# Lukeasargen/Show-Attend-and-Tell-Pytorch-Lightning

Hardware: AMD Instinct MI355X
Metric: captions/sec (train step) at B=128, 256px, seq_len=22 (higher is better)
Workload: dtype bf16; 1 GPU; C2: resnet50 encoder_size=7 encoder_dim=512 vocab=6400 T=22, 128 images/GPU x R=5 captions, trainable encoder, Adam, full lengths, decoder_tf=always; global_batch_images=128, parallelism=dp1, grad_bucket_dtype=fp32

## Files before the change

show-attend-and-tell-pytorch-lightning_amd/csrc/api.hip:

```cpp
#include <stdarg.h>

#include "../../include/sat_hip.h"
#include "decoder.h"
#include "gemm.h"
#include "gemm_bf16_common.h"
#include "temperature.h"
#include "caption_score.h"

namespace sat {
static thread_local char g_err[512] = {0};
int& dev_switch(int which) {
    static int v[SW_COUNT] = {0 , getenv("SAT_NO_WGRAD3X3") ? !atoi(getenv("SAT_NO_WGRAD3X3")) : 1,
                              getenv("SAT_REDUCE_Z16") ? atoi(getenv("SAT_REDUCE_Z16")) : 1, getenv("SAT_WIDE_TILES") ? atoi(getenv("SAT_WIDE_TILES")) : 0,
                              getenv("SAT_BN_ONEPASS") ? atoi(getenv("SAT_BN_ONEPASS")) : 1,
                              getenv("SAT_BN_VPT") ? atoi(getenv("SAT_BN_VPT")) : 2,
                              getenv("SAT_ACC_PREFETCH") ? atoi(getenv("SAT_ACC_PREFETCH")) : 0};
    return v[which];
}
int& trace_launches() { static int on = getenv("SAT_TRACE_LAUNCH") ? 1 : 0; return on; }
char* last_error_buf() { return g_err; }
int fail(int code, const char* fmt, ...) {
    va_list ap; va_start(ap, fmt); vsnprintf(g_err, sizeof g_err, fmt, ap); va_end(ap);
    return code;
}
}

using namespace sat;

extern "C" {

int sat_abi_version(void) { return SAT_HIP_ABI_VERSION; }
int sat_debug_trace_launches(int32_t on) { sat::trace_launches() = on ? 1 : 0; return SAT_OK; }
int sat_debug_option(const char* name, int32_t value) {
    if (!name) return fail(SAT_EINVAL, "debug_option: null name");
    if (!strcmp(name, "wgrad3x3")) { dev_switch(SW_WGRAD3X3) = value; return SAT_OK; }
    if (!strcmp(name, "reduce_z16")) { dev_switch(SW_REDUCE_Z16) = value; return SAT_OK; }
    if (!strcmp(name, "acc_prefetch")) { dev_switch(SW_ACC_PREFETCH) = value; return SAT_OK; }
    if (!strcmp(name, "bn_vpt")) { dev_switch(SW_BN_VPT) = value; return SAT_OK; }
    if (!strcmp(name, "bn_onepass")) { dev_switch(SW_BN_ONEPASS) = value; return SAT_OK; }
    if (!strcmp(name, "wide_tiles")) { dev_switch(SW_WIDE_TILES) = value; return SAT_OK; }
    if (!strcmp(name, "glds_tile")) { glds_force_tile() = value; return SAT_OK; }
    if (!strcmp(name, "glds_stages8")) { glds_stages8() = value; return SAT_OK; }
    if (!strcmp(name, "glds_tall_k")) { glds_tall_k() = value; return SAT_OK; }
    if (!strcmp(name, "glds_tall_conv")) { glds_tall_conv() = value; return SAT_OK; }
    if (!strcmp(name, "tile_override")) { gemm_tile_override() = value; return SAT_OK; }
    return fail(SAT_EINVAL, "debug_option: unknown option %s", name);
}
const char* sat_last_error(void) { return last_error_buf(); }

static int gemm_from_desc(const sat_gemm_desc* d, const sat_gemm_types* t, void* stream);
int sat_gemm_f32(const sat_gemm_desc* d, void* stream) { return gemm_from_desc(d, nullptr, stream); }
int sat_gemm_ex(const sat_gemm_desc* d, const sat_gemm_types* t, void* stream) {
    if (!t) return fail(SAT_EINVAL, "sat_gemm_ex: null type descriptor");
    return gemm_from_desc(d, t, stream);
}
static int gemm_from_desc(const sat_gemm_desc* d, const sat_gemm_types* t, void* stream) {
    if (!d) return fail(SAT_EINVAL, "sat_gemm_f32: null descriptor");
    if (d->amode != A_ROW && d->amode != A_KMAJOR) return fail(SAT_EINVAL, "sat_gemm_f32: amode %d (dense modes only)", d->amode);
    if (d->bmode != B_ROW && d->bmode != B_KMAJOR) return fail(SAT_EINVAL, "sat_gemm_f32: bmode %d (dense modes only)", d->bmode);
    GemmArgs g;
    g.A = d->A; g.lda = d->lda; g.a_rows = d->a_rows; g.B = d->B; g.ldb = d->ldb; g.C = d->C; g.ldc = d->ldc; g.c_rows = d->c_rows;
    g.M = d->M; g.N = d->N; g.K = d->K; g.amode = d->amode; g.bmode = d->bmode; g.accumulate = d->accumulate; g.epi = d->epi;
    g.bias = d->bias; g.e0 = d->e0; g.lde0 = d->lde0; g.c0 = d->c0; g.c1 = d->c1; g.slab = d->slab; g.slab_elems = d->slab_elems;
    if (t) { g.a_bf16 = t->a_bf16; g.b_bf16 = t->b_bf16; g.c_bf16 = t->c_bf16; g.bf16_mfma = t->bf16_mfma; }
    return launch_gemm(g, (hipStream_t)stream);
}

size_t sat_decoder_workspace_bytes(const sat_decoder_dims* d) {
    if (check_dims(d) != SAT_OK) return 0;
    return decoder_workspace_bytes(*d);
}

static int check_params(const sat_decoder_dims* d, const sat_decoder_params* w, const char* what) {
    if (!w) return fail(SAT_EINVAL, "%s: null parameter struct", what);
    if (!w->embedding || !w->init_f_w || !w->init_f_b || !w->init_i_w || !w->init_i_b || !w->w_ih || !w->w_hh || !w->b_ih || !w->b_hh ||
        !w->att_enc || !w->att_dec || !w->att_f || !w->beta_w || !w->beta_b || !w->out_hidden || !w->out_w)
        return fail(SAT_EINVAL, "%s: null tensor in parameter struct", what);
    if (d->deep_output && !w->out_context) return fail(SAT_EINVAL, "%s: deep output needs output.context.weight", what);
    for (int l = 1; l < d->layers; ++l)
        if (!w->up_w_ih[l - 1] || !w->up_w_hh[l - 1] || !w->up_b_ih[l - 1] || !w->up_b_hh[l - 1])
            return fail(SAT_EINVAL, "%s: null tensor for LSTM layer %d", what, l);
    return SAT_OK;
}
static int check_batch(const sat_decoder_batch* b) {
    if (!b || !b->ann || !b->caps || !b->lengths || !b->prow || !b->src_row || !b->step_offsets_host || !b->teacher_host)
        return fail(SAT_EINVAL, "decoder: null field in batch struct");
    return SAT_OK;
}

int sat_decoder_train_fwd(const sat_decoder_dims* d, const sat_decoder_params* w, const sat_decoder_batch* b, float* logits_packed,
                          float* alphas, void* workspace, size_t workspace_bytes, void* stream) {
    SAT_TRY(check_dims(d)); SAT_TRY(check_params(d, w, "decoder_train_fwd")); SAT_TRY(check_batch(b));
    if (!alphas || !workspace || (d->P > 0 && !logits_packed)) return fail(SAT_EINVAL, "decoder_train_fwd: null output/workspace");
    return decoder_fwd(*d, *w, *b, logits_packed, alphas, (char*)workspace, workspace_bytes, (hipStream_t)stream);
}

int sat_decoder_train_bwd(const sat_decoder_dims* d, const sat_decoder_params* w, const sat_decoder_batch* b, const float* dlogits_packed,
                          const float* alphas, const float* dalphas, const sat_decoder_params* g, float* dann, void* workspace,
                          size_t workspace_bytes, void* stream) {
    SAT_TRY(check_dims(d)); SAT_TRY(check_params(d, w, "decoder_train_bwd")); SAT_TRY(check_params(d, g, "decoder_train_bwd(grads)")); SAT_TRY(check_batch(b));
    if (!alphas || !dann || !workspace || (d->P > 0 && !dlogits_packed)) return fail(SAT_EINVAL, "decoder_train_bwd: null input/output/workspace");
    return decoder_bwd(*d, *w, *b, dlogits_packed, alphas, dalphas, *g, dann, (char*)workspace, workspace_bytes, (hipStream_t)stream);
}

int sat_ce_label_smooth_fwd(const float* logits, const int32_t* targets, int32_t P, int32_t V, float smoothing, float* lse_rows,
                            float* loss_rows, int32_t* correct_rows, float* out, void* stream) {
    if (!logits || !targets || !lse_rows || !loss_rows || !correct_rows || !out) return fail(SAT_EINVAL, "ce_label_smooth_fwd: null pointer");
    return ce_fwd(logits, targets, P, V, smoothing, lse_rows, loss_rows, correct_rows, out, (hipStream_t)stream);
}
int sat_ce_label_smooth_bwd(const float* logits, const int32_t* targets, const float* lse_rows, int32_t P, int32_t V, float smoothing,
                            const float* gscale, float* dlogits, void* stream) {
    if (!logits || !targets || !lse_rows || !dlogits) return fail(SAT_EINVAL, "ce_label_smooth_bwd: null pointer");
    return ce_bwd(logits, targets, lse_rows, P, V, smoothing, gscale, dlogits, (hipStream_t)stream);
}
int sat_doubly_stochastic_fwd(const float* alphas, int32_t N, int32_t T1, int32_t L, float gamma, float* asum, float* part, float* out, void* stream) {
    if (!alphas || !asum || !part || !out) return fail(SAT_EINVAL, "doubly_stochastic_fwd: null pointer");
    return ds_fwd(alphas, N, T1, L, gamma, asum, part, out, (hipStream_t)stream);
}
int sat_doubly_stochastic_bwd(const float* asum, const float* gscale, int32_t N, int32_t T1, int32_t L, float gamma, float* dalphas, void* stream) {
    if (!asum || !dalphas) return fail(SAT_EINVAL, "doubly_stochastic_bwd: null pointer");
    return ds_bwd(asum, gscale, N, T1, L, gamma, dalphas, (hipStream_t)stream);
}

size_t sat_temperature_workspace_bytes(int32_t P, int32_t V) {
    if (P <= 0 || V <= 0) { fail(SAT_EINVAL, "temperature_workspace_bytes: non-positive size (P=%d V=%d)", P, V); return 0; }
    return temperature_workspace_bytes(P, V);
}
int sat_temperature_nll(const float* logits, const int32_t* targets, int32_t P, int32_t V, const float* temperatures, int32_t n_temperatures,
// ... 460 lines not shown
```

show-attend-and-tell-pytorch-lightning_amd/csrc/encoder.hip:

```cpp
#include <stdlib.h>
#include "../../include/sat_hip.h"
#include "common.h"
#include "gemm.h"
#include "profile.h"

namespace sat {

typedef __bf16 bf16x4 __attribute__((ext_vector_type(4)));
template <typename T> __device__ __forceinline__ float4 ld4(const T* p, long i4);
template <> __device__ __forceinline__ float4 ld4<float>(const float* p, long i4) { return reinterpret_cast<const float4*>(p)[i4]; }
template <> __device__ __forceinline__ float4 ld4<__bf16>(const __bf16* p, long i4) {
    bf16x4 v = reinterpret_cast<const bf16x4*>(p)[i4];
    return make_float4((float)v[0], (float)v[1], (float)v[2], (float)v[3]);
}
template <typename T> __device__ __forceinline__ void st4(T* p, long i4, float4 v);
template <> __device__ __forceinline__ void st4<float>(float* p, long i4, float4 v) { reinterpret_cast<float4*>(p)[i4] = v; }
template <> __device__ __forceinline__ void st4<__bf16>(__bf16* p, long i4, float4 v) {
    bf16x4 o; o[0] = (__bf16)v.x; o[1] = (__bf16)v.y; o[2] = (__bf16)v.z; o[3] = (__bf16)v.w;
    reinterpret_cast<bf16x4*>(p)[i4] = o;
}

__global__ void cast_f32_bf16_kernel(const float* __restrict__ src, __bf16* __restrict__ dst, long n4) {
    long e = (long)blockIdx.x * blockDim.x + threadIdx.x;
    if (e < n4) st4<__bf16>(dst, e, reinterpret_cast<const float4*>(src)[e]);
}
__global__ void normalize_nhwc8_bf16_kernel(const float* __restrict__ img, __bf16* __restrict__ out, int H, int W, long total,
                                            float m0, float m1, float m2, float s0, float s1, float s2) {
    long e = (long)blockIdx.x * blockDim.x + threadIdx.x;
    if (e >= total) return;
    long hw = (long)H * W; long n = e / hw, p = e - n * hw;
    const float* src = img + n * 3 * hw + p;
    st4<__bf16>(out, 2 * e, make_float4((src[0] - m0) / s0, (src[hw] - m1) / s1, (src[2 * hw] - m2) / s2, 0.f));
    st4<__bf16>(out, 2 * e + 1, make_float4(0.f, 0.f, 0.f, 0.f));
}
__global__ void pad_c3_to_c8_bf16_kernel(const float* __restrict__ w3, __bf16* __restrict__ w8, long n) {
    long e = (long)blockIdx.x * blockDim.x + threadIdx.x;
    if (e >= n) return;
    st4<__bf16>(w8, 2 * e, make_float4(w3[3 * e], w3[3 * e + 1], w3[3 * e + 2], 0.f));
    st4<__bf16>(w8, 2 * e + 1, make_float4(0.f, 0.f, 0.f, 0.f));
}
__global__ void unpad_c8_to_c3_kernel(const float* __restrict__ w8, float* __restrict__ w3, long n) {
    long e = (long)blockIdx.x * blockDim.x + threadIdx.x;
    if (e >= n) return;
    w3[3 * e] = w8[8 * e]; w3[3 * e + 1] = w8[8 * e + 1]; w3[3 * e + 2] = w8[8 * e + 2];
}

__global__ void normalize_nhwc4_padded_bf16_kernel(const float* __restrict__ img, __bf16* __restrict__ out, int H, int W, long total,
                                                   float m0, float m1, float m2, float s0, float s1, float s2) {
    long e = (long)blockIdx.x * blockDim.x + threadIdx.x;
    if (e >= total) return;
    const int Wp = W + 6, Hp = H + 6;
    const unsigned eu = (unsigned)e;
    const int xp = (int)(eu % Wp); const unsigned t = eu / Wp; const int yp = (int)(t % Hp); const long n = t / Hp;
    const int x = xp - 3, y = yp - 3;
    float4 v = make_float4(0.f, 0.f, 0.f, 0.f);
    if ((unsigned)x < (unsigned)W && (unsigned)y < (unsigned)H) {
        const long hw = (long)H * W; const float* src = img + n * 3 * hw + (long)y * W + x;
        v = make_float4((src[0] - m0) / s0, (src[hw] - m1) / s1, (src[2 * hw] - m2) / s2, 0.f);
    }
    st4<__bf16>(out, e, v);
}
__global__ void stem_filter_pairs_kernel(const float* __restrict__ w3, __bf16* __restrict__ wp, long n) {
    long e = (long)blockIdx.x * blockDim.x + threadIdx.x;
    if (e >= n) return;
    const int sp = (int)(e % 4); const long kr = e / 4;
    const float* a = w3 + (kr * 7 + 2 * sp) * 3;
    st4<__bf16>(wp, 2 * e, make_float4(a[0], a[1], a[2], 0.f));
    st4<__bf16>(wp, 2 * e + 1, sp < 3 ? make_float4(a[3], a[4], a[5], 0.f) : make_float4(0.f, 0.f, 0.f, 0.f));
}
__global__ void stem_filter_grad_unpairs_kernel(const float* __restrict__ dwp, float* __restrict__ dw3, long n) {
    long e = (long)blockIdx.x * blockDim.x + threadIdx.x;
    if (e >= n) return;
    const int s = (int)(e % 7); const long kr = e / 7;
    const float* a = dwp + ((kr * 4 + (s >> 1)) * 8 + (s & 1) * 4);
    dw3[3 * e] = a[0]; dw3[3 * e + 1] = a[1]; dw3[3 * e + 2] = a[2];
}

__global__ void normalize_nhwc4_kernel(const float* __restrict__ img, float* __restrict__ out, int H, int W, long total,
                                       float m0, float m1, float m2, float s0, float s1, float s2) {
    long e = (long)blockIdx.x * blockDim.x + threadIdx.x;
    if (e >= total) return;
    long hw = (long)H * W; long n = e / hw, p = e - n * hw;
    const float* src = img + n * 3 * hw + p;
    float4 v;
    v.x = (src[0] - m0) / s0; v.y = (src[hw] - m1) / s1; v.z = (src[2 * hw] - m2) / s2; v.w = 0.f;
    reinterpret_cast<float4*>(out)[e] = v;
// ... 740 lines not shown
    if (V == 4) reinterpret_cast<float4*>(y)[e] = make_float4(s[0], s[1], s[2], s[3]);
    else y[e] = s[0];
}
__device__ __forceinline__ void bilinear_src(int o, int in, int out, int& i0, int& i1, float& l1) {
    float s = ((float)o + 0.5f) * ((float)in / (float)out) - 0.5f;
    if (s < 0.f) s = 0.f;
    i0 = (int)s; i1 = i0 + (i0 < in - 1 ? 1 : 0); l1 = s - (float)i0;
}
__global__ void bilinear_fwd_kernel(const float* __restrict__ x, float* __restrict__ y, int H, int W, int C, int P, int Q, long total) {
    long e = (long)blockIdx.x * blockDim.x + threadIdx.x;
    if (e >= total) return;
    const unsigned eu = (unsigned)e; int c = (int)(eu % C); unsigned t = eu / C; int q = (int)(t % Q); t /= Q; int p = (int)(t % P); long n = t / P;
    int h0, h1, w0, w1; float lh, lw;
    bilinear_src(p, H, P, h0, h1, lh); bilinear_src(q, W, Q, w0, w1, lw);
    const float* b = x + n * H * W * C + c;
    float v00 = b[((long)h0 * W + w0) * C], v01 = b[((long)h0 * W + w1) * C], v10 = b[((long)h1 * W + w0) * C], v11 = b[((long)h1 * W + w1) * C];
    y[e] = (1.f - lh) * ((1.f - lw) * v00 + lw * v01) + lh * ((1.f - lw) * v10 + lw * v11);
}
__global__ void bilinear_bwd_kernel(const float* __restrict__ dy, float* __restrict__ dx, int H, int W, int C, int P, int Q, long total) {
    long e = (long)blockIdx.x * blockDim.x + threadIdx.x;
    if (e >= total) return;
    const unsigned eu = (unsigned)e; int c = (int)(eu % C); unsigned t = eu / C; int w = (int)(t % W); t /= W; int h = (int)(t % H); long n = t / H;
    float s = 0.f;
    for (int p = 0; p < P; ++p) {
        int h0, h1; float lh; bilinear_src(p, H, P, h0, h1, lh);
        float wh = (h0 == h ? 1.f - lh : 0.f) + (h1 == h ? lh : 0.f);
        if (wh == 0.f) continue;
        for (int q = 0; q < Q; ++q) {
            int w0, w1; float lw; bilinear_src(q, W, Q, w0, w1, lw);
            float ww = (w0 == w ? 1.f - lw : 0.f) + (w1 == w ? lw : 0.f);
            if (ww != 0.f) s += wh * ww * dy[((n * P + p) * Q + q) * C + c];
        }
    }
    dx[e] = s;
}

template <typename T>
__global__ void grouped_filter_expand_kernel(const T* __restrict__ wg, T* __restrict__ wd, int K, int C, int RS, int groups) {
    const long e = (long)blockIdx.x * blockDim.x + threadIdx.x;
    const long total = (long)K * RS * C;
    if (e >= total) return;
    const int c = (int)(e % C); const long t = e / C; const int rs = (int)(t % RS), k = (int)(t / RS);
    const int cg = C / groups, kg = K / groups;
    const int g = k / kg;
    const int cl = c - g * cg;
    wd[e] = (cl >= 0 && cl < cg) ? wg[((long)k * RS + rs) * cg + cl] : (T)0.f;
}
__global__ void grouped_filter_grad_extract_kernel(const float* __restrict__ dwd, float* __restrict__ dwg, int K, int C, int RS, int groups) {
    const long e = (long)blockIdx.x * blockDim.x + threadIdx.x;
    const int cg = C / groups, kg = K / groups;
    const long total = (long)K * RS * cg;
    if (e >= total) return;
    const int cl = (int)(e % cg); const long t = e / cg; const int rs = (int)(t % RS), k = (int)(t / RS);
    dwg[e] = dwd[((long)k * RS + rs) * C + (k / kg) * cg + cl];
}

}

using namespace sat;

static int conv_geom(const sat_conv_geom* g, ConvGeom& o, int vec = 4) {
    SAT_REQUIRE(g, "conv: null geometry");
    o.N = g->N; o.H = g->H; o.W = g->W; o.C = g->C; o.K = g->K; o.R = g->R; o.S = g->S; o.stride = g->stride; o.pad = g->pad; o.sw = (g->stride_w > 0 && g->stride_w != g->stride) ? g->stride_w : 0;
    SAT_REQUIRE(o.N > 0 && o.H > 0 && o.W > 0 && o.C > 0 && o.K > 0 && o.R > 0 && o.S > 0 && o.stride > 0 && o.pad >= 0, "conv: bad geometry");
    o.P = (o.H + 2 * o.pad - o.R) / o.stride + 1; o.Q = (o.W + 2 * o.pad - o.S) / (o.sw ? o.sw : o.stride) + 1;
    SAT_REQUIRE(o.P > 0 && o.Q > 0, "conv: empty output");
    SAT_REQUIRE(o.C % vec == 0 && o.K % vec == 0, "conv: C=%d and K=%d must be multiples of %d (pad the stem channels)", o.C, o.K, vec);
    return SAT_OK;
}

extern "C" {

static int conv_fwd_any(const void* x, const void* w, const float* bias, void* y, const sat_conv_geom* geom, int bf16, void* stream,
                        float* tile_stats = nullptr, int* tile_rows = nullptr) {
    ConvGeom g; SAT_TRY(conv_geom(geom, g, bf16 ? 8 : 4));
    if (!x || !w || !y) return fail(SAT_EINVAL, "conv2d_fwd: null pointer");
    GemmArgs a; a.a_bf16 = a.b_bf16 = a.c_bf16 = a.bf16_mfma = bf16;
    a.M = g.N * g.P * g.Q; a.N = g.K; a.K = g.R * g.S * g.C;
    a.B = w; a.ldb = a.K; a.bmode = B_ROW; a.C = y; a.ldc = g.K; a.g = g;
    if (g.R == 1 && g.S == 1 && g.stride == 1 && g.pad == 0) { a.A = x; a.lda = g.C; a.amode = A_ROW; }
    else { a.A = x; a.amode = A_CONV_FWD; }
    if (bias) { a.epi = EPI_BIAS; a.bias = bias; }
    a.tile_stats = tile_stats; a.tile_rows = tile_rows;
    return launch_gemm(a, (hipStream_t)stream);
}
int sat_conv2d_fwd(const float* x, const float* w, const float* bias, float* y, const sat_conv_geom* geom, void* stream) {
    return conv_fwd_any(x, w, bias, y, geom, 0, stream);
}
int sat_conv2d_fwd_bf16(const void* x, const void* w, const float* bias, void* y, const sat_conv_geom* geom, void* stream) {
    return conv_fwd_any(x, w, bias, y, geom, 1, stream);
}
size_t sat_conv2d_fwd_stats_bytes(const sat_conv_geom* geom) {
    ConvGeom g; if (conv_geom(geom, g, 8) != SAT_OK) return 0;
    return (size_t)cdiv((long)g.N * g.P * g.Q, 64L) * g.K * 2 * sizeof(float);
}
int sat_conv2d_fwd_bf16_stats(const void* x, const void* w, void* y, const sat_conv_geom* geom, float* tile_stats, int32_t* tile_rows, void* stream) {
    if (!tile_stats || !tile_rows) return fail(SAT_EINVAL, "conv2d_fwd_bf16_stats: null statistics buffer");
    int tr = 0;
    SAT_TRY(conv_fwd_any(x, w, nullptr, y, geom, 1, stream, tile_stats, &tr));
    *tile_rows = tr;
    return SAT_OK;
}

struct BnBwdStats { const void* x; const unsigned char* mask; const float* mean; const float* invstd; float* tile_stats; int* tile_rows; };
static int conv_dgrad_any(const void* dy, const void* w, void* dx, const sat_conv_geom* geom, int accumulate, int bf16, void* stream,
                          const BnBwdStats* bs = nullptr, const void* add_src = nullptr, const uint8_t* add_mask = nullptr) {
    ConvGeom g; SAT_TRY(conv_geom(geom, g, bf16 ? 8 : 4));
    if (!dy || !w || !dx) return fail(SAT_EINVAL, "conv2d_dgrad: null pointer");
    GemmArgs a; a.a_bf16 = a.b_bf16 = a.c_bf16 = a.bf16_mfma = bf16;
    a.accumulate = accumulate; a.C = dx; a.ldc = g.C; a.g = g;
    if (add_src) {
        SAT_REQUIRE(bf16 && g.stride == 1, "conv2d_dgrad: add_src needs bf16 storage and stride 1");
        a.accumulate = 1; a.add_src = add_src; a.add_mask = add_mask;
    }
    if (bs) {
        *bs->tile_rows = 0;
        if (bf16 && !(g.stride == 2)) {
            a.bn_x = bs->x; a.bn_mask = bs->mask; a.bn_mean = bs->mean; a.bn_invstd = bs->invstd; a.tile_stats = bs->tile_stats; a.tile_rows = bs->tile_rows;
        }
    }
    if (g.R == 1 && g.S == 1 && g.stride == 1 && g.pad == 0) {
        a.M = g.N * g.H * g.W; a.N = g.C; a.K = g.K; a.A = dy; a.lda = g.K; a.amode = A_ROW; a.B = w; a.ldb = g.C; a.bmode = B_KMAJOR;
    } else if (bf16 && g.stride == 2) {
        a.A = dy; a.amode = A_CONV_DGRAD; a.B = w; a.bmode = B_CONV_DGRAD_W; a.N = g.C;
        for (int ph = 0; ph < 2; ++ph)
            for (int pw = 0; pw < 2; ++pw) {
                ConvGeom c = g; c.cls = 1; c.ph = ph; c.pw = pw;
                c.Hc = (g.H - ph + 1) / 2; c.Wc = (g.W - pw + 1) / 2;
                c.r0 = (ph + g.pad) & 1; c.s0 = (pw + g.pad) & 1;
                c.rc = c.r0 < g.R ? (g.R - c.r0 + 1) / 2 : 0; c.sc = c.s0 < g.S ? (g.S - c.s0 + 1) / 2 : 0;
                if (c.Hc <= 0 || c.Wc <= 0) continue;
                a.g = c; a.M = g.N * c.Hc * c.Wc; a.K = c.rc * c.sc * g.K;
                if (a.K == 0 && accumulate) continue;
                if (c.sc == 0) a.g.sc = 1;
                SAT_TRY(launch_gemm(a, (hipStream_t)stream));
            }
        return SAT_OK;
    } else {
        a.M = g.N * g.H * g.W; a.N = g.C; a.K = g.R * g.S * g.K; a.A = dy; a.amode = A_CONV_DGRAD; a.B = w; a.bmode = B_CONV_DGRAD_W;
    }
    return launch_gemm(a, (hipStream_t)stream);
}
int sat_conv2d_dgrad(const float* dy, const float* w, float* dx, const sat_conv_geom* geom, int accumulate, void* stream) {
    return conv_dgrad_any(dy, w, dx, geom, accumulate, 0, stream);
}
int sat_conv2d_dgrad_bf16(const void* dy, const void* w, void* dx, const sat_conv_geom* geom, int accumulate, void* stream) {
    return conv_dgrad_any(dy, w, dx, geom, accumulate, 1, stream);
}
int sat_conv2d_dgrad_bf16_fused(const void* dy, const void* w, void* dx, const sat_conv_geom* geom, const void* add_src, const uint8_t* add_mask, const void* bn_x,
                                const uint8_t* bn_relu_mask, const float* bn_mean, const float* bn_invstd, float* tile_stats, int32_t* tile_rows, void* stream) {
    if (!add_src) return fail(SAT_EINVAL, "conv2d_dgrad_bf16_fused: null add_src (use sat_conv2d_dgrad_bf16[_bnstats])");
    if (!bn_x) return conv_dgrad_any(dy, w, dx, geom, 1, 1, stream, nullptr, add_src, add_mask);
    if (!bn_mean || !bn_invstd || !tile_stats || !tile_rows) return fail(SAT_EINVAL, "conv2d_dgrad_bf16_fused: null statistics pointer");
    int tr = 0;
    BnBwdStats bs{bn_x, bn_relu_mask, bn_mean, bn_invstd, tile_stats, &tr};
    SAT_TRY(conv_dgrad_any(dy, w, dx, geom, 1, 1, stream, &bs, add_src, add_mask));
    *tile_rows = tr;
    return SAT_OK;
}
size_t sat_conv2d_dgrad_stats_bytes(const sat_conv_geom* geom) {
    ConvGeom g; if (conv_geom(geom, g, 8) != SAT_OK) return 0;
    return (size_t)cdiv((long)g.N * g.H * g.W, 64L) * g.C * 2 * sizeof(float);
}
int sat_conv2d_dgrad_bf16_bnstats(const void* dy, const void* w, void* dx, const sat_conv_geom* geom, int accumulate, const void* bn_x, const uint8_t* bn_relu_mask,
                                  const float* bn_mean, const float* bn_invstd, float* tile_stats, int32_t* tile_rows, void* stream) {
    if (!bn_x || !bn_mean || !bn_invstd || !tile_stats || !tile_rows) return fail(SAT_EINVAL, "conv2d_dgrad_bf16_bnstats: null pointer");
    int tr = 0;
    BnBwdStats bs{bn_x, bn_relu_mask, bn_mean, bn_invstd, tile_stats, &tr};
    SAT_TRY(conv_dgrad_any(dy, w, dx, geom, accumulate, 1, stream, &bs));
    *tile_rows = tr;
    return SAT_OK;
}

static int conv_wgrad_any(const void* dy, const void* x, float* dw, const sat_conv_geom* geom, float* slab, int64_t slab_elems, int bf16, void* stream) {
    ConvGeom g; SAT_TRY(conv_geom(geom, g, bf16 ? 8 : 4));
    if (!dy || !x || !dw) return fail(SAT_EINVAL, "conv2d_wgrad: null pointer");
    if (bf16 && wgrad3x3_eligible(g)) return launch_wgrad3x3(dy, x, dw, g, slab, (long)slab_elems, (hipStream_t)stream);
    GemmArgs a; a.a_bf16 = a.b_bf16 = a.bf16_mfma = bf16; a.c_bf16 = 0;
    a.M = g.K; a.N = g.R * g.S * g.C; a.K = g.N * g.P * g.Q;
    a.A = dy; a.lda = g.K; a.amode = A_KMAJOR; a.C = dw; a.ldc = a.N; a.g = g; a.slab = slab; a.slab_elems = slab_elems;
    if (g.R == 1 && g.S == 1 && g.stride == 1 && g.pad == 0) { a.B = x; a.ldb = g.C; a.bmode = B_KMAJOR; }
    else { a.B = x; a.bmode = B_CONV_WGRAD; }
    return launch_gemm(a, (hipStream_t)stream);
}
int sat_conv2d_wgrad(const float* dy, const float* x, float* dw, const sat_conv_geom* geom, float* slab, int64_t slab_elems, void* stream) {
    return conv_wgrad_any(dy, x, dw, geom, slab, slab_elems, 0, stream);
}
int sat_conv2d_wgrad_bf16(const void* dy, const void* x, float* dw, const sat_conv_geom* geom, float* slab, int64_t slab_elems, void* stream) {
    return conv_wgrad_any(dy, x, dw, geom, slab, slab_elems, 1, stream);
}

size_t sat_conv2d_wgrad_slab_bytes(const sat_conv_geom* geom) {
    ConvGeom g; if (conv_geom(geom, g) != SAT_OK) return 0;
    return gemm_slab_bytes(g.K, g.R * g.S * g.C, g.N * g.P * g.Q);
}

int sat_image_normalize_nhwc4(const float* img_nchw, float* out_nhwc4, int32_t N, int32_t H, int32_t W, const float* mean3_host, const float* std3_host, void* stream) {
    if (!img_nchw || !out_nhwc4 || !mean3_host || !std3_host) return fail(SAT_EINVAL, "image_normalize: null pointer");
    long total = (long)N * H * W;
    hipLaunchKernelGGL(normalize_nhwc4_kernel, dim3(cdiv(total, 256)), dim3(256), 0, (hipStream_t)stream, img_nchw, out_nhwc4, H, W, total,
                       mean3_host[0], mean3_host[1], mean3_host[2], std3_host[0], std3_host[1], std3_host[2]);
    return launch_ok("normalize_nhwc4");
}

int sat_pad_channels_3to4(const float* src, float* dst, int64_t pixels, int32_t inverse, void* stream) {
// ... 444 lines not shown
```

Measured before the change: 32500 captions/s.

## Add persistent streaming kernel for large-M narrow 1x1 convolutions

Adds a specialized persistent kernel for bf16 1x1 convolutions with small K and N (at most 256). It keeps the whole weight matrix resident in LDS, streams 128-row tiles of activations per wave with register prefetch of the next tile, and fuses the forward BN tile statistics, dgrad accumulate/add, and BN-backward statistics epilogues. Forward and dgrad 1x1 paths try it first and otherwise fall back to the generic GEMM. It targets the re-loading of weights and per-tile overhead in memory-bound early ResNet layers, at the cost of a large new code path with its own numerics and occupancy tuning.

Result: no change. 32580 captions/s, median of 5 (+0.2%).

```diff
diff --git a/show-attend-and-tell-pytorch-lightning_amd/csrc/api.hip b/show-attend-and-tell-pytorch-lightning_amd/csrc/api.hip
--- a/show-attend-and-tell-pytorch-lightning_amd/csrc/api.hip
+++ b/show-attend-and-tell-pytorch-lightning_amd/csrc/api.hip
@@ -3,6 +3,7 @@
 #include "../../include/sat_hip.h"
 #include "decoder.h"
 #include "gemm.h"
+#include "conv1x1_stream.h"
 #include "gemm_bf16_common.h"
 #include "temperature.h"
 #include "caption_score.h"
@@ -44,6 +45,8 @@
     if (!strcmp(name, "glds_tall_k")) { glds_tall_k() = value; return SAT_OK; }
     if (!strcmp(name, "glds_tall_conv")) { glds_tall_conv() = value; return SAT_OK; }
     if (!strcmp(name, "tile_override")) { gemm_tile_override() = value; return SAT_OK; }
+    if (!strcmp(name, "conv1x1_stream")) { conv1x1_stream_mode() = value; return SAT_OK; }
+    if (!strcmp(name, "conv1x1_stream_grid")) { conv1x1_stream_grid_cap() = value; return SAT_OK; }
     return fail(SAT_EINVAL, "debug_option: unknown option %s", name);
 }
 const char* sat_last_error(void) { return last_error_buf(); }
diff --git a/show-attend-and-tell-pytorch-lightning_amd/csrc/conv1x1_stream.h b/show-attend-and-tell-pytorch-lightning_amd/csrc/conv1x1_stream.h
--- /dev/null
+++ b/show-attend-and-tell-pytorch-lightning_amd/csrc/conv1x1_stream.h
@@ -0,0 +1,10 @@
+#pragma once
+#include "gemm.h"
+
+namespace sat {
+
+int conv1x1_stream_try(const GemmArgs& g, hipStream_t st);
+int& conv1x1_stream_mode();
+int& conv1x1_stream_grid_cap();
+
+}
diff --git a/show-attend-and-tell-pytorch-lightning_amd/csrc/conv1x1_stream.hip b/show-attend-and-tell-pytorch-lightning_amd/csrc/conv1x1_stream.hip
--- /dev/null
+++ b/show-attend-and-tell-pytorch-lightning_amd/csrc/conv1x1_stream.hip
@@ -0,0 +1,347 @@
+#include <stdlib.h>
+
+#include "conv1x1_stream.h"
+#include "gemm_bf16_common.h"
+#include "profile.h"
+
+namespace sat {
+
+struct SArgs {
+    const __bf16* A; long lda;
+    const __bf16* W; long ldw;
+    __bf16* C; long ldc;
+    int M, N, K;
+    int accumulate;
+    const __bf16* add_src; const unsigned char* add_mask;
+    const __bf16* bn_x; const unsigned char* bn_mask; const float* bn_mean; const float* bn_invstd;
+    float* tile_stats;
+    int stat_rows;
+    int rotate;
+    int nch;
+};
+
+__device__ __forceinline__ bf16x8 ld16(const __bf16* p) { return *reinterpret_cast<const bf16x8*>(p); }
+__device__ __forceinline__ bf16x8 zero8() { const uint4 z = make_uint4(0, 0, 0, 0); return __builtin_bit_cast(bf16x8, z); }
+
+constexpr int S_LDC = 64 + 8;
+constexpr size_t stream_lds_bytes(int ks, int nch, int waves) { return (size_t)ks * 2 * nch * 1024 + (size_t)waves * 32 * S_LDC * 2; }
+
+template <int KS, int NCHT, bool DG, bool BNS>
+__global__ __launch_bounds__(512) void conv1x1_stream_kernel(SArgs a) {
+    constexpr int LDC = S_LDC, T = KS / 4, NJ = 4;
+    extern __shared__ __attribute__((aligned(16))) __bf16 smem[];
+    const int lane = threadIdx.x & 63, wave = threadIdx.x >> 6, nwv = blockDim.x >> 6, li = lane & 31, lh = lane >> 5;
+    const int nch = NCHT ? NCHT : a.nch, ncb = 2 * nch;
+    __bf16* wl = smem;
+    __bf16* cs = smem + (size_t)KS * ncb * 512 + wave * (32 * LDC);
+    const int ntiles = (a.M + 127) >> 7;
+
+    for (int f = wave; f < KS * ncb; f += nwv) {
+        const int s = f / ncb, cb = f - s * ncb;
+        const int n = cb * 32 + li, k = s * 16 + lh * 8;
+        bf16x8 v = zero8();
+        if (n < a.N && k < a.K) {
+            if constexpr (!DG) v = ld16(a.W + (long)n * a.ldw + k);
+            else {
+#pragma unroll
+                for (int e = 0; e < 8; ++e) v[e] = a.W[(long)(k + e) * a.ldw + n];
+            }
+        }
+        *reinterpret_cast<bf16x8*>(wl + ((size_t)f * 64 + lane) * 8) = v;
+    }
+    __syncthreads();
+
+    auto load_a = [&](bf16x8 (&af)[KS], int tile, int rb) {
+        const int row = tile * 128 + rb * 32 + li;
+#pragma unroll
+        for (int s = 0; s < KS; ++s) {
+            const int k = s * 16 + lh * 8;
+            af[s] = (row < a.M && k < a.K) ? ld16(a.A + (long)row * a.lda + k) : zero8();
+        }
+    };
+
+    const int seg = lane & 7, lrow0 = lane >> 3;
+    const bool fwd_stats = !DG && a.tile_stats != nullptr;
+    const int seg_rbs = a.stat_rows >> 5;
+    float s1[BNS ? NJ : 1][8], s2[BNS ? NJ : 1][8];
+    bf16x8 af[KS];
+
+    auto block = [&](int tile, int rb, int chunk, float (&fs)[2][4], bool load_next, int ntile, int nrb) {
+        const int rowbase = tile * 128 + rb * 32, c0 = chunk * 64, col = c0 + seg * 8;
+        f32x16 acc[2];
+#pragma unroll
+        for (int c = 0; c < 2; ++c)
+#pragma unroll
+            for (int r = 0; r < 16; ++r) acc[c][r] = 0.f;
+        const int rot = (T > 1 && a.rotate) ? ((chunk * 5 + (rowbase / a.stat_rows) * 3) & (T - 1)) : 0;
+        const __bf16* wc = wl + ((size_t)(chunk * 2) * 64 + lane) * 8;
+#pragma unroll
+        for (int r0 = 0; r0 < T; ++r0) {
+            if (rot != r0) continue;
+#pragma unroll
+            for (int t = 0; t < T; ++t) {
+                const int kt = (r0 + t) % T;
+#pragma unroll
+                for (int s = 0; s < 4; ++s)
+#pragma unroll
+                    for (int c = 0; c < 2; ++c) {
+                        const bf16x8 w = ld16(wc + ((size_t)(kt * 4 + s) * ncb + c) * 512);
+                        acc[c] = __builtin_amdgcn_mfma_f32_32x32x16_bf16(af[kt * 4 + s], w, acc[c], 0, 0, 0);
+                    }
+            }
+        }
+        if (load_next) load_a(af, ntile, nrb);
+        bf16x8 oldv[DG ? NJ : 1], bxv[BNS ? NJ : 1]; unsigned mbv[DG ? NJ : 1], bmv[BNS ? NJ : 1];
+        float mu[8];
+        if constexpr (DG) {
+#pragma unroll
+            for (int j = 0; j < NJ; ++j) {
+                const int row = rowbase + lrow0 + 8 * j;
+                const bool ok = row < a.M && col < a.N;
+                const long off = ok ? (long)row * a.ldc + col : 0;
+                oldv[j] = zero8(); mbv[j] = 0;
+                if (a.accumulate && ok) {
+                    oldv[j] = ld16((a.add_src ? a.add_src : a.C) + off);
+                    mbv[j] = a.add_mask ? (unsigned)a.add_mask[off >> 3] : 0xFFu;
+                }
+                if constexpr (BNS) {
+                    bxv[j] = zero8(); bmv[j] = 0;
+                    if (ok) { bxv[j] = ld16(a.bn_x + off); bmv[j] = a.bn_mask ? (unsigned)a.bn_mask[off >> 3] : 0xFFu; }
+                }
+            }
+            if constexpr (BNS) {
+#pragma unroll
+                for (int e = 0; e < 8; ++e) mu[e] = (col + e < a.N) ? a.bn_mean[col + e] : 0.f;
+            }
+        }
+        if constexpr (!DG) {
+            if (fwd_stats) {
+                const bool t128 = seg_rbs == 4;
+                const bool seg_start = t128 ? !(rb & 1) : true, seg_end = t128 ? (rb & 1) : true;
+                const int half = t128 ? (rb >> 1) : (rb & 1);
+#pragma unroll
+                for (int c = 0; c < 2; ++c) {
+                    float q1 = seg_start ? 0.f : fs[c][0], q2 = seg_start ? 0.f : fs[c][1];
+#pragma unroll
+                    for (int r = 0; r < 16; ++r) {
+                        const int row = rowbase + (r & 3) + 8 * (r >> 2) + 4 * lh;
+                        const float vb = (float)(__bf16)acc[c][r];
+                        if (row < a.M) { q1 += vb; q2 = fmaf(vb, vb, q2); }
+                    }
+                    fs[c][0] = q1; fs[c][1] = q2;
+                    if (seg_end) {
+                        q1 += __shfl_xor(q1, 32, 64); q2 += __shfl_xor(q2, 32, 64);
+                        if (half == 0) { fs[c][2] = q1; fs[c][3] = q2; }
+                        else {
+                            const int stile = t128 ? tile : tile * 2 + (rb >> 1);
+                            const int n = c0 + c * 32 + li;
+                            if (lh == 0 && n < a.N && (long)stile * a.stat_rows < a.M) {
+                                float* o = a.tile_stats + ((long)stile * a.N + n) * 2;
+                                o[0] = fs[c][2] + q1; o[1] = fs[c][3] + q2;
+                            }
+                        }
+                    }
+                }
+            }
+        }
+        const bool odd = lane & 1;
+#pragma unroll
+        for (int c = 0; c < 2; ++c)
+#pragma unroll
+            for (int r = 0; r < 16; r += 2) {
+                const int lr0 = (r & 3) + 8 * (r >> 2) + 4 * lh, lc = c * 32 + li;
+                const float v0 = acc[c][r], v1 = acc[c][r + 1];
+                const float give = odd ? v0 : v1;
+                const float got = __int_as_float(__builtin_amdgcn_mov_dpp(__float_as_int(give), 0xB1 , 0xF, 0xF, true));
+                typedef __bf16 bf16x2 __attribute__((ext_vector_type(2)));
+                bf16x2 pk;
+                if (odd) { pk[0] = (__bf16)got; pk[1] = (__bf16)v1; } else { pk[0] = (__bf16)v0; pk[1] = (__bf16)got; }
+                *reinterpret_cast<bf16x2*>(cs + (lr0 + (odd ? 1 : 0)) * LDC + (lc & ~1)) = pk;
+            }
+        asm volatile("s_waitcnt lgkmcnt(0)" ::: "memory");
+        if constexpr (BNS) {
+            if (rb % seg_rbs == 0) {
+#pragma unroll
+                for (int j = 0; j < NJ; ++j)
+#pragma unroll
+                    for (int e = 0; e < 8; ++e) { s1[j][e] = 0.f; s2[j][e] = 0.f; }
+            }
+        }
+#pragma unroll
+        for (int j = 0; j < NJ; ++j) {
+            const int lrow = lrow0 + 8 * j, row = rowbase + lrow;
+            if (row < a.M && col < a.N) {
+                bf16x8 o = ld16(cs + lrow * LDC + seg * 8);
+                if constexpr (DG) {
+                    if (a.accumulate) {
+#pragma unroll
+                        for (int e = 0; e < 8; ++e) o[e] = (__bf16)((float)o[e] + (((mbv[j] >> e) & 1u) ? (float)oldv[j][e] : 0.f));
+                    }
+                }
+                *reinterpret_cast<bf16x8*>(a.C + (long)row * a.ldc + col) = o;
+                if constexpr (BNS) {
+#pragma unroll
+                    for (int e = 0; e < 8; ++e) {
+                        const float gv = ((bmv[j] >> e) & 1u) ? (float)o[e] : 0.f;
+                        s1[j][e] += gv; s2[j][e] = fmaf(gv, (float)bxv[j][e] - mu[e], s2[j][e]);
+                    }
+                }
+            }
+        }
+        asm volatile("" ::: "memory");
+        if constexpr (BNS) {
+            if (rb % seg_rbs == seg_rbs - 1) {
+                float t1[8], t2[8];
+#pragma unroll
+                for (int e = 0; e < 8; ++e) { t1[e] = 0.f; t2[e] = 0.f; }
+#pragma unroll
+                for (int j = 0; j < NJ; ++j)
+#pragma unroll
+                    for (int e = 0; e < 8; ++e) {
+                        float v1 = s1[j][e], v2 = s2[j][e];
+#pragma unroll
+                        for (int o = 8; o < 64; o <<= 1) { v1 += __shfl_xor(v1, o, 64); v2 += __shfl_xor(v2, o, 64); }
+                        t1[e] += v1; t2[e] += v2;
+                    }
+                const int stile = (seg_rbs == 4) ? tile : tile * 2 + (rb >> 1);
+                if (lane < 8 && col < a.N && (long)stile * a.stat_rows < a.M) {
+#pragma unroll
+                    for (int e = 0; e < 8; ++e) {
+                        float* o = a.tile_stats + ((long)stile * a.N + col + e) * 2;
+                        o[0] = t1[e]; o[1] = t2[e] * a.bn_invstd[col + e];
+                    }
+                }
+            }
+        }
+    };
+
+    const int tstride = (int)gridDim.x * nwv;
+    int tile = (int)blockIdx.x * nwv + wave;
+    if (tile >= ntiles) return;
+    load_a(af, tile, 0);
+    for (; tile < ntiles; tile += tstride) {
+        const bool more = tile + tstride < ntiles;
+        if constexpr (BNS) {
+            float fs[2][4];
+#pragma unroll 1
+            for (int it = 0; it < 4 * nch; ++it) {
+                const int chunk = it >> 2, rb = it & 3;
+                const bool last = it + 1 == 4 * nch;
+                block(tile, rb, chunk, fs, !last || more, last ? tile + tstride : tile, (rb + 1) & 3);
+            }
+        } else if constexpr (NCHT != 0) {
+            float fs[NCHT][2][4];
+#pragma unroll 1
+            for (int rb = 0; rb < 4; ++rb) {
+#pragma unroll
+                for (int chunk = 0; chunk < NCHT; ++chunk) {
+                    const bool nxt = chunk + 1 == NCHT;
+                    block(tile, rb, chunk, fs[chunk], nxt && (rb < 3 || more), rb < 3 ? tile : tile + tstride, (rb + 1) & 3);
+                }
+            }
+        } else {
+            float fs[2][4];
+#pragma unroll 1
+            for (int it = 0; it < 4 * nch; ++it) {
+                const int rb = it / nch, chunk = it - rb * nch;
+                const bool nxt = chunk + 1 == nch;
+                block(tile, rb, chunk, fs, nxt && (rb < 3 || more), rb < 3 ? tile : tile + tstride, (rb + 1) & 3);
+            }
+        }
+    }
+}
+
+int& conv1x1_stream_mode() { static int v = getenv("SAT_CONV1X1_STREAM") ? atoi(getenv("SAT_CONV1X1_STREAM")) : 1; return v; }
+int& conv1x1_stream_grid_cap() { static int v = 0; return v; }
+static int conv1x1_stream_min_rows() { static const int v = getenv("SAT_CONV1X1_STREAM_MIN_ROWS") ? atoi(getenv("SAT_CONV1X1_STREAM_MIN_ROWS")) : 262144; return v; }
+
+static inline bool al16p(const void* p) { return (reinterpret_cast<uintptr_t>(p) & 15) == 0; }
+
+template <int KS, int NCHT, bool DG, bool BNS>
+static int run_stream(const SArgs& s, const char* pname, double flops, double bytes, hipStream_t st) {
+    const void* fn = reinterpret_cast<const void*>(&conv1x1_stream_kernel<KS, NCHT, DG, BNS>);
+    static bool attr_set = false;
+    if (!attr_set) { SAT_CHECK_HIP(hipFuncSetAttribute(fn, hipFuncAttributeMaxDynamicSharedMemorySize, 160 * 1024 - 512)); attr_set = true; }
+    const int ntiles = cdiv(s.M, 128);
+    const int nwv = ntiles >= 2048 ? 8 : (ntiles >= 512 ? 4 : 2);
+    const size_t lds = stream_lds_bytes(KS, s.nch, nwv);
+    static int c_nwv = 0, c_resident = 0; static size_t c_lds = 0;
+    if (c_nwv != nwv || c_lds != lds) {
+        int dev = 0, cus = 0, per_cu = 0;
+        SAT_CHECK_HIP(hipGetDevice(&dev));
+        SAT_CHECK_HIP(hipDeviceGetAttribute(&cus, hipDeviceAttributeMultiprocessorCount, dev));
+        SAT_CHECK_HIP(hipOccupancyMaxActiveBlocksPerMultiprocessor(&per_cu, fn, 64 * nwv, lds));
+        c_resident = (cus > 0 ? cus : 1) * (per_cu > 0 ? per_cu : 1); c_nwv = nwv; c_lds = lds;
+    }
+    const int groups = cdiv(ntiles, nwv);
+    const int cap = conv1x1_stream_grid_cap() > 0 ? conv1x1_stream_grid_cap() : c_resident;
+    const int rounds = cdiv(groups, cap);
+    const int grid = cdiv(groups, rounds);
+    ProfScope prof(pname, flops, bytes, st);
+    hipLaunchKernelGGL((conv1x1_stream_kernel<KS, NCHT, DG, BNS>), dim3(grid), dim3(64 * nwv), lds, st, s);
+    return launch_ok("conv1x1_stream_kernel");
+}
+
+int conv1x1_stream_try(const GemmArgs& g, hipStream_t st) {
+    const int mode = conv1x1_stream_mode();
+    if (!mode) return -1;
+    if (!(g.a_bf16 && g.b_bf16 && g.c_bf16 && g.bf16_mfma)) return -1;
+    if (g.amode != A_ROW || g.a_rows || g.c_rows || g.epi != EPI_NONE || g.slab || g.g.cls) return -1;
+    const bool dg = g.bmode == B_KMAJOR;
+    if (!dg && g.bmode != B_ROW) return -1;
+    if (dg && mode == 3) return -1;
+    if (g.M <= 0 || g.N <= 0 || g.K <= 0 || g.K % 8 || g.N % 8 || (long)g.K * g.N > 32768 || g.K > 256 || g.N > 256) return -1;
+    if (g.K > 64 && g.K % 64 == 0 && g.K != 128 && g.K != 256) return -1;
+    if (g.lda % 8 || g.ldb % 8 || g.ldc % 8 || !al16p(g.A) || !al16p(g.B) || !al16p(g.C)) return -1;
+    if (mode != 2 && (g.M < conv1x1_stream_min_rows() || g.K > 64)) return -1;
+    if (gemm_tile_override() > 0 || glds_force_tile() >= 0 || dev_switch(SW_WIDE_TILES) || getenv("SAT_NO_GLDS") || getenv("SAT_GLDS_ROT") || getenv("SAT_GLDS_TALL") ||
+        getenv("SAT_TILES128_MIN")) return -1;
+    const bool glds = g.K % 64 == 0;
+    const long tiles128 = (long)cdiv(g.M, 128) * cdiv(g.N, 128);
+    const int stat_rows = ((g.N >= 128 && g.M >= 128 && tiles128 >= 512) || (glds && g.N <= 64 && g.M >= 8192)) ? 128 : 64;
+    bool stats = false;
+    if (!dg) {
+        if (g.accumulate || g.add_src || g.bn_x) return -1;
+        stats = g.tile_stats && g.tile_rows;
+    } else {
+        if (g.add_src && (!g.accumulate || !al16p(g.add_src))) return -1;
+        if (g.bn_x) {
+            if (!(g.tile_stats && g.tile_rows && g.bn_mean && g.bn_invstd && g.ldc == g.N && al16p(g.bn_x) && glds && g.K <= 128)) return -1;
+            stats = true;
+        } else if (g.tile_stats) return -1;
+    }
+    const int KS = g.K <= 64 ? 4 : (g.K <= 128 ? 8 : 16), nch = cdiv(g.N, 64);
+    if (!dg && nch == 3) return -1;
+    if (stream_lds_bytes(KS, nch, 8) > 160 * 1024 - 512) return -1;
+    SArgs s;
+    s.A = reinterpret_cast<const __bf16*>(g.A); s.lda = g.lda; s.W = reinterpret_cast<const __bf16*>(g.B); s.ldw = g.ldb;
+    s.C = reinterpret_cast<__bf16*>(g.C); s.ldc = g.ldc; s.M = g.M; s.N = g.N; s.K = g.K; s.accumulate = g.accumulate;
+    s.add_src = reinterpret_cast<const __bf16*>(g.add_src); s.add_mask = g.add_mask;
+    s.bn_x = reinterpret_cast<const __bf16*>(g.bn_x); s.bn_mask = g.bn_mask; s.bn_mean = g.bn_mean; s.bn_invstd = g.bn_invstd;
+    s.tile_stats = stats ? g.tile_stats : nullptr; s.stat_rows = stat_rows; s.rotate = glds ? 1 : 0; s.nch = nch;
+    if (g.tile_rows) *g.tile_rows = stats ? stat_rows : 0;
+    char pname[128];
+    if (profile_enabled()) {
+        static const bool shapes = getenv("SAT_PROFILE_SHAPES") != nullptr;
+        if (shapes) snprintf(pname, sizeof pname, "gemm_stream1x1_%s M%d N%d K%d acc%d join%d bn%d", dg ? "nn" : "nt", g.M, g.N, g.K, g.accumulate, g.add_src ? 1 : 0, g.bn_x ? 1 : 0);
+        else snprintf(pname, sizeof pname, "gemm_stream1x1_%s", dg ? "nn" : "nt");
+    }
+    const double mn = (double)g.M * g.N;
+    double bytes = 2.0 * g.M * g.K + 2.0 * g.N * g.K + 2.0 * mn;
+    if (g.accumulate) bytes += 2.0 * mn + (g.add_mask ? mn / 8 : 0.0);
+    if (g.bn_x) bytes += 2.0 * mn + (g.bn_mask ? mn / 8 : 0.0);
+    if (stats) bytes += 8.0 * cdiv(g.M, stat_rows) * g.N;
+    const double flops = 2.0 * mn * g.K;
+    const bool bn = g.bn_x != nullptr;
+#define SAT_SCASE(KSV, NCHV, DGV, BNV) \
+    if (KS == KSV && dg == DGV && bn == BNV && (NCHV == 0 || nch == NCHV)) return run_stream<KSV, NCHV, DGV, BNV>(s, pname, flops, bytes, st);
+    SAT_SCASE(4, 1, false, false) SAT_SCASE(4, 2, false, false) SAT_SCASE(4, 4, false, false)
+    SAT_SCASE(8, 1, false, false) SAT_SCASE(8, 2, false, false) SAT_SCASE(8, 4, false, false)
+    SAT_SCASE(16, 1, false, false) SAT_SCASE(16, 2, false, false)
+    SAT_SCASE(4, 0, true, false) SAT_SCASE(8, 0, true, false) SAT_SCASE(16, 0, true, false)
+    SAT_SCASE(4, 0, true, true) SAT_SCASE(8, 0, true, true)
+#undef SAT_SCASE
+    return -1;
+}
+
+}
diff --git a/show-attend-and-tell-pytorch-lightning_amd/csrc/encoder.hip b/show-attend-and-tell-pytorch-lightning_amd/csrc/encoder.hip
--- a/show-attend-and-tell-pytorch-lightning_amd/csrc/encoder.hip
+++ b/show-attend-and-tell-pytorch-lightning_amd/csrc/encoder.hip
@@ -2,6 +2,7 @@
 #include "../../include/sat_hip.h"
 #include "common.h"
 #include "gemm.h"
+#include "conv1x1_stream.h"
 #include "profile.h"
 
 namespace sat {
@@ -908,6 +909,10 @@
     else { a.A = x; a.amode = A_CONV_FWD; }
     if (bias) { a.epi = EPI_BIAS; a.bias = bias; }
     a.tile_stats = tile_stats; a.tile_rows = tile_rows;
+    if (a.amode == A_ROW) {
+        const int r = conv1x1_stream_try(a, (hipStream_t)stream);
+        if (r != -1) return r;
+    }
     return launch_gemm(a, (hipStream_t)stream);
 }
 int sat_conv2d_fwd(const float* x, const float* w, const float* bias, float* y, const sat_conv_geom* geom, void* stream) {
@@ -947,6 +952,8 @@
     }
     if (g.R == 1 && g.S == 1 && g.stride == 1 && g.pad == 0) {
         a.M = g.N * g.H * g.W; a.N = g.C; a.K = g.K; a.A = dy; a.lda = g.K; a.amode = A_ROW; a.B = w; a.ldb = g.C; a.bmode = B_KMAJOR;
+        const int r = conv1x1_stream_try(a, (hipStream_t)stream);
+        if (r != -1) return r;
     } else if (bf16 && g.stride == 2) {
         a.A = dy; a.amode = A_CONV_DGRAD; a.B = w; a.bmode = B_CONV_DGRAD_W; a.N = g.C;
         for (int ph = 0; ph < 2; ++ph)
```
